# zhouxinlzu/PebbleSDR

Hardware: AMD Instinct MI355X
Metric: IQ Msamples/s through full ProcessBlock chain (higher is better)
Workload: dtype f32; 1 GPU; configs[1]: 20 Msps int8-shape IQ (values k/128, resident in HBM as float2), 1 channel/GPU, mixer+decimate(D=64)+WFM mono demod + 8192-bin SignalSpectrum per 2048-sample frame; frames_per_buffer=2048, spectrum_bins=8192, parallelism=independent channel per GPU, no collectives

## Files before the change

### pebblesdr_amd/csrc/fft_lds.h

```cpp
#pragma once
#include "common.h"

namespace pg {

__device__ __forceinline__ int lpad(int i) { return i + ((i >> 5) << 2); }
__device__ __forceinline__ int lpad4(int i) { return i + (i >> 4); }
__device__ __forceinline__ int lpad1(int i) { return i + (i >> 5); }
enum { kPad4per32 = 0, kPad1per16 = 1, kPad1per32 = 2 };
template <int A> __device__ __forceinline__ int lpad_sel(int i) { return A == kPad1per16 ? lpad4(i) : A == kPad1per32 ? lpad1(i) : lpad(i); }
template <int N> struct FftLds { static constexpr int kSlots = N + (N >> 5) * 4; };

__host__ __device__ constexpr int fft_passes(int n) { return n == 8192 ? 5 : 4; }
__host__ __device__ constexpr int fft_radix(int n, int pass) { return n == 2048 ? (pass == 0 ? 4 : 8) : n == 4096 ? 8 : (pass == 0 ? 2 : 8); }
__host__ __device__ constexpr int fft_tw_off(int n, int P)
{
    int off = 0, p = 1;
    for (int i = 0; i < fft_passes(n); i++) {
        if (p == P) return off;
        if (p > 1) off += 3 * p;
        p *= fft_radix(n, i);
    }
    return off;
}

template <int DIR> __device__ __forceinline__ float2 mul_mj(float2 a)
{
    return DIR > 0 ? make_float2(a.y, -a.x) : make_float2(-a.y, a.x);
}
template <int DIR> __device__ __forceinline__ float2 twid(float2 w)
{
    return DIR > 0 ? w : make_float2(w.x, -w.y);
}

template <int DIR> __device__ __forceinline__ void bfly2(float2 *u)
{
    float2 a = u[0], b = u[1];
    u[0] = cadd(a, b);
    u[1] = csub(a, b);
}
template <int DIR> __device__ __forceinline__ float2 add_mj(float2 a, float2 b)
{
    return cswap(b) * make_float2((float)DIR, (float)-DIR) + a;
}
template <int DIR> __device__ __forceinline__ float2 sub_mj(float2 a, float2 b)
{
    return cswap(b) * make_float2((float)-DIR, (float)DIR) + a;
}
template <int DIR> __device__ __forceinline__ void bfly4(float2 *u)
{
    float2 t0 = cadd(u[0], u[2]), t1 = csub(u[0], u[2]);
    float2 t2 = cadd(u[1], u[3]), d = csub(u[1], u[3]);
    u[0] = cadd(t0, t2);
    u[2] = csub(t0, t2);
    u[1] = add_mj<DIR>(t1, d);
    u[3] = sub_mj<DIR>(t1, d);
}
template <int DIR> __device__ __forceinline__ void bfly8(float2 *u)
{
    float2 e[4] = {u[0], u[2], u[4], u[6]};
    float2 o[4] = {u[1], u[3], u[5], u[7]};
    bfly4<DIR>(e);
    bfly4<DIR>(o);
    const float c = 0.70710678118654752440f;
    const float2 o1 = cscale(add_mj<DIR>(o[1], o[1]), c);
    const float2 o3 = cscale(sub_mj<DIR>(o[3], o[3]), c);
    u[0] = cadd(e[0], o[0]); u[4] = csub(e[0], o[0]);
    u[1] = cadd(e[1], o1);   u[5] = csub(e[1], o1);
    u[2] = add_mj<DIR>(e[2], o[2]); u[6] = sub_mj<DIR>(e[2], o[2]);
    u[3] = csub(e[3], o3);   u[7] = cadd(e[3], o3);
}
__host__ __device__ constexpr int perm32(int k) { return 4 * (k & 7) + (k >> 3); }
__device__ __forceinline__ void dft32(float2 *u)
{
    constexpr float kC[22] = {1.f, 0.98078528040323044913f, 0.92387953251128675613f, 0.83146961230254523708f, 0.70710678118654752440f,
                              0.55557023301960222474f, 0.38268343236508977173f, 0.19509032201612826785f, 0.f, -0.19509032201612826785f,
                              -0.38268343236508977173f, -0.55557023301960222474f, -0.70710678118654752440f, -0.83146961230254523708f,
                              -0.92387953251128675613f, -0.98078528040323044913f, -1.f, -0.98078528040323044913f, -0.92387953251128675613f,
                              -0.83146961230254523708f, -0.70710678118654752440f, -0.55557023301960222474f};
    constexpr float kS[22] = {0.f, -0.19509032201612826785f, -0.38268343236508977173f, -0.55557023301960222474f, -0.70710678118654752440f,
                              -0.83146961230254523708f, -0.92387953251128675613f, -0.98078528040323044913f, -1.f, -0.98078528040323044913f,
                              -0.92387953251128675613f, -0.83146961230254523708f, -0.70710678118654752440f, -0.55557023301960222474f,
                              -0.38268343236508977173f, -0.19509032201612826785f, 0.f, 0.19509032201612826785f, 0.38268343236508977173f,
                              0.55557023301960222474f, 0.70710678118654752440f, 0.83146961230254523708f};
#pragma unroll
    for (int nb = 0; nb < 4; nb++) {
        float2 t[8];
#pragma unroll
        for (int na = 0; na < 8; na++) t[na] = u[nb + 4 * na];
        bfly8<+1>(t);
#pragma unroll
        for (int ka = 0; ka < 8; ka++) {
            const int m = nb * ka;
            u[4 * ka + nb] = m == 0 ? t[ka] : m == 8 ? mul_mj<+1>(t[ka]) : cmul(make_float2(kC[m], kS[m]), t[ka]);
        }
    }
#pragma unroll
    for (int ka = 0; ka < 8; ka++) bfly4<+1>(u + 4 * ka);
}

template <int R, int DIR> __device__ __forceinline__ void bfly(float2 *u)
{
    if (R == 2) bfly2<DIR>(u);
    else if (R == 4) bfly4<DIR>(u);
    else bfly8<DIR>(u);
}

template <int T> __device__ __forceinline__ void fft_sync()
{
    if (T == 64) wave_sync();
    else __syncthreads();
}

template <int N, int T, int R, int P, int DIR, bool FIRST, bool LAST>
__device__ __forceinline__ void fft_pass(float2 (&x)[N / T], float2 *lds, const float2 *__restrict__ tw, int tid)
{
    constexpr int E = N / T, Q = E / R;
    static_assert(E % R == 0 && Q >= 1, "points per work-item must be a multiple of the radix");
    constexpr int PAD_IN = (!FIRST && P == 4) ? kPad1per16 : (!FIRST && T == 64 && P == 32) ? kPad1per32 : kPad4per32;
    constexpr int PAD_OUT = (FIRST && R == 4) ? kPad1per16 : kPad4per32;
    float2 w1 = make_float2(1.f, 0.f), w2 = w1, w4 = w1;
    auto fetch_tw = [&](int k) {
        if (T == 64) opaque(k);
        const float2 *t = tw + fft_tw_off(N, P) + k;
        w1 = twid<DIR>(t[0]);
        if (R >= 4) w2 = twid<DIR>(t[P]);
        if (R == 8) w4 = twid<DIR>(t[2 * P]);
    };
    if (P > 1) fetch_tw(tid & (P - 1));
    if (!FIRST) {
        {
            const float2 *rp = lds + lpad_sel<PAD_IN>(tid);
#pragma unroll
            for (int q = 0; q < Q; q += 2) {
#pragma unroll
                for (int r = 0; r < R; r++) {
                    x[q + r * Q] = rp[lpad_sel<PAD_IN>(T * (q + r * Q))];
                    if (q + 1 < Q) x[q + 1 + r * Q] = rp[lpad_sel<PAD_IN>(T * (q + 1 + r * Q))];
                }
                if (T == 64) sched_fence();
            }
        }
        fft_sync<T>();
    }
    const int jbase = (P <= T) ? (tid - (tid & (P - 1))) * R + (tid & (P - 1)) : tid;
    float2 *wbase = lds + lpad_sel<PAD_OUT>(jbase);
#pragma unroll
    for (int q = 0; q < Q; q++) {
        const int b = tid + T * q;
        float2 u[R];
#pragma unroll
        for (int r = 0; r < R; r++) u[r] = x[q + r * Q];
        const int k = b & (P - 1);
        if (P > 1) {
            if (P > T && q > 0) fetch_tw(k);
            u[1] = cmul(w1, u[1]);
            if (R >= 4) {
                const float2 w3 = cmul(w1, w2);
                u[2] = cmul(w2, u[2]);
                u[3] = cmul(w3, u[3]);
                if (R == 8) {
                    u[4] = cmul(w4, u[4]);
                    u[5] = cmul(cmul(w4, w1), u[5]);
                    u[6] = cmul(cmul(w4, w2), u[6]);
                    u[7] = cmul(cmul(w4, w3), u[7]);
                }
            }
        }
        bfly<R, DIR>(u);
        if (LAST) {
#pragma unroll
            for (int r = 0; r < R; r++) x[q + r * Q] = u[r];
        } else {
            const int cq = (P <= T) ? T * R * q : R * (T * q - (T * q) % P) + (T * q) % P;
            float2 *wp = wbase + lpad_sel<PAD_OUT>(cq);
#pragma unroll
            for (int r = 0; r < R; r++) wp[lpad_sel<PAD_OUT>(r * P)] = u[r];
        }
        if (T == 64) sched_fence();
    }
    if (!LAST) fft_sync<T>();
}

__device__ __forceinline__ void fft_first32(float2 (&x)[32], float2 *lds, int tid)
{
    dft32(x);
    float2 *wp = lds + lpad1(32 * tid);
#pragma unroll
    for (int k = 0; k < 32; k++) wp[k] = x[perm32(k)];
    wave_sync();
}

template <int N, int DIR, int T = 256>
__device__ __forceinline__ void fft_regs(float2 (&x)[N / T], float2 *lds, const float2 *__restrict__ tw, int tid)
{
    static_assert((T == 256 && (N == 2048 || N == 4096 || N == 8192)) || (T == 64 && N == 2048), "supported sizes");
    if (N == 2048 && T == 64) {
        static_assert(!(N == 2048 && T == 64) || DIR == +1, "the wave transform is forward only");
        fft_first32(reinterpret_cast<float2 (&)[32]>(x), lds, tid);
        fft_pass<N, T, 8, 32, DIR, false, false>(x, lds, tw, tid);
        fft_pass<N, T, 8, 256, DIR, false, true>(x, lds, tw, tid);
    } else if (N == 2048) {
        fft_pass<N, T, 4, 1, DIR, true, false>(x, lds, tw, tid);
        fft_pass<N, T, 8, 4, DIR, false, false>(x, lds, tw, tid);
        fft_pass<N, T, 8, 32, DIR, false, false>(x, lds, tw, tid);
        fft_pass<N, T, 8, 256, DIR, false, true>(x, lds, tw, tid);
    } else if (N == 4096) {
        fft_pass<N, T, 8, 1, DIR, true, false>(x, lds, tw, tid);
        fft_pass<N, T, 8, 8, DIR, false, false>(x, lds, tw, tid);
        fft_pass<N, T, 8, 64, DIR, false, false>(x, lds, tw, tid);
        fft_pass<N, T, 8, 512, DIR, false, true>(x, lds, tw, tid);
    } else {
        fft_pass<N, T, 2, 1, DIR, true, false>(x, lds, tw, tid);
        fft_pass<N, T, 8, 2, DIR, false, false>(x, lds, tw, tid);
        fft_pass<N, T, 8, 16, DIR, false, false>(x, lds, tw, tid);
        fft_pass<N, T, 8, 128, DIR, false, false>(x, lds, tw, tid);
        fft_pass<N, T, 8, 1024, DIR, false, true>(x, lds, tw, tid);
    }
}

}
```

### pebblesdr_amd/csrc/fft_t128.h

```cpp
#pragma once
#include "fft_lds.h"

namespace pg {

constexpr int kTw128B = 0, kTw128C = 48, kTw128Count = 48 + 512;

__host__ __device__ constexpr int perm16(int k) { return 4 * (k & 3) + (k >> 2); }

__device__ __forceinline__ void dft16(float2 *u)
{
    constexpr float kC[10] = {1.f, 0.92387953251128675613f, 0.70710678118654752440f, 0.38268343236508977173f, 0.f,
                              -0.38268343236508977173f, -0.70710678118654752440f, -0.92387953251128675613f, -1.f, -0.92387953251128675613f};
    constexpr float kS[10] = {0.f, -0.38268343236508977173f, -0.70710678118654752440f, -0.92387953251128675613f, -1.f,
                              -0.92387953251128675613f, -0.70710678118654752440f, -0.38268343236508977173f, 0.f, 0.38268343236508977173f};
#pragma unroll
    for (int nb = 0; nb < 4; nb++) {
        float2 t[4];
#pragma unroll
        for (int na = 0; na < 4; na++) t[na] = u[nb + 4 * na];
        bfly4<+1>(t);
#pragma unroll
        for (int ka = 0; ka < 4; ka++) {
            const int m = nb * ka;
            u[4 * ka + nb] = m == 0 ? t[ka] : m == 4 ? mul_mj<+1>(t[ka]) : cmul(make_float2(kC[m], kS[m]), t[ka]);
        }
    }
#pragma unroll
    for (int ka = 0; ka < 4; ka++) bfly4<+1>(u + 4 * ka);
}

struct Tw128Regs {
    float2 b1, b2, b4, c1, c2, c4, c8;
    float2 cx[16];
};
__device__ __forceinline__ void tw128_fill_cx(Tw128Regs &w)
{
    w.cx[0] = make_float2(1.f, 0.f);
    w.cx[1] = w.c1; w.cx[2] = w.c2; w.cx[3] = cmul_pk(w.c1, w.c2); w.cx[4] = w.c4;
    w.cx[5] = cmul_pk(w.c4, w.c1); w.cx[6] = cmul_pk(w.c4, w.c2); w.cx[7] = cmul_pk(w.c4, w.cx[3]); w.cx[8] = w.c8;
#pragma unroll
    for (int i = 1; i < 8; i++) w.cx[8 + i] = cmul_pk(w.c8, w.cx[i]);
}

template <class Sync, bool DO_LDS = true, bool DO_MATH = true, bool REGS = false, bool FULLC = false, int HELD = 0>
__device__ __forceinline__ void fft2048_t128(float2 (&x)[16], float2 *lds, const float2 *__restrict__ tw, int t, Sync sync, Tw128Regs wr = Tw128Regs())
{
    if (DO_MATH) dft16(x);
    if (DO_LDS) {
        float2 *wp = lds + lpad4(16 * t);
#pragma unroll
        for (int k = 0; k < 16; k++) wp[k] = x[perm16(k)];
    }
    sync();
    {
        const int k = t & 15;
        float2 w1, w2, w4;
        if (REGS) { w1 = wr.b1; w2 = wr.b2; w4 = wr.b4; }
        else { w1 = tw[kTw128B + k]; w2 = tw[kTw128B + 16 + k]; w4 = tw[kTw128B + 32 + k]; }
        if (DO_LDS) {
            const float2 *rp = lds + lpad4(t);
#pragma unroll
            for (int m = 0; m < 16; m++) x[m] = rp[136 * m];
        }
        sync();
        const float2 w3 = cmul_pk(w1, w2), w5 = cmul_pk(w4, w1), w6 = cmul_pk(w4, w2), w7 = cmul_pk(w4, w3);
        float2 *wbase = lds + lpad((t - k) * 8 + k);
#pragma unroll
        for (int q = 0; q < 2; q++) {
            float2 u[8];
#pragma unroll
            for (int r = 0; r < 8; r++) u[r] = x[q + 2 * r];
            if (DO_MATH) {
                u[1] = cmul_pk(w1, u[1]); u[2] = cmul_pk(w2, u[2]); u[3] = cmul_pk(w3, u[3]); u[4] = cmul_pk(w4, u[4]);
                u[5] = cmul_pk(w5, u[5]); u[6] = cmul_pk(w6, u[6]); u[7] = cmul_pk(w7, u[7]);
                bfly8<+1>(u);
            }
            float2 *wp = wbase + lpad(1024 * q);
            if (DO_LDS) {
#pragma unroll
                for (int r = 0; r < 8; r++) wp[lpad(16 * r)] = u[r];
            } else {
#pragma unroll
                for (int r = 0; r < 8; r++) x[q + 2 * r] = u[r];
            }
        }
    }
    sync();
    {
        float2 w1, w2, w4, w8;
        if (REGS) { w1 = wr.c1; w2 = wr.c2; w4 = wr.c4; w8 = wr.c8; }
        else { w1 = tw[kTw128C + t]; w2 = tw[kTw128C + 128 + t]; w4 = tw[kTw128C + 256 + t]; w8 = tw[kTw128C + 384 + t]; }
        if (DO_LDS) {
            const float2 *rp = lds + lpad(t);
#pragma unroll
            for (int m = 0; m < 16; m++) x[m] = rp[144 * m];
        }
        sync();
        if (!DO_MATH) return;
        if (REGS && FULLC) {
#pragma unroll
            for (int m = 1; m < 16; m++) x[m] = cmul_pk(wr.cx[m], x[m]);
        } else {
        const float2 w3 = cmul_pk(w1, w2), w5 = cmul_pk(w4, w1), w6 = cmul_pk(w4, w2), w7 = cmul_pk(w4, w3);
        x[1] = cmul_pk(w1, x[1]); x[2] = cmul_pk(w2, x[2]); x[3] = cmul_pk(w3, x[3]); x[4] = cmul_pk(w4, x[4]);
        x[5] = cmul_pk(w5, x[5]); x[6] = cmul_pk(w6, x[6]); x[7] = cmul_pk(w7, x[7]); x[8] = cmul_pk(w8, x[8]);
        x[9] = cmul_pk(REGS && HELD >= 1 ? wr.cx[9] : cmul_pk(w8, w1), x[9]);
        x[10] = cmul_pk(REGS && HELD >= 2 ? wr.cx[10] : cmul_pk(w8, w2), x[10]);
        x[11] = cmul_pk(REGS && HELD >= 3 ? wr.cx[11] : cmul_pk(w8, w3), x[11]);
        x[12] = cmul_pk(REGS && HELD >= 4 ? wr.cx[12] : cmul_pk(w8, w4), x[12]);
        x[13] = cmul_pk(REGS && HELD >= 5 ? wr.cx[13] : cmul_pk(w8, w5), x[13]);
        x[14] = cmul_pk(REGS && HELD >= 6 ? wr.cx[14] : cmul_pk(w8, w6), x[14]);
        x[15] = cmul_pk(REGS && HELD >= 7 ? wr.cx[15] : cmul_pk(w8, w7), x[15]);
        }
        dft16(x);
        float2 y[16];
#pragma unroll
        for (int r = 0; r < 16; r++) y[r] = x[perm16(r)];
#pragma unroll
        for (int r = 0; r < 16; r++) x[r] = y[r];
    }
}

}
```

### pebblesdr_amd/csrc/kernels_spectrum.h

```cpp
#pragma once
#include "fft_lds.h"
#include "fft_t128.h"
#include "fft_w64.h"
#include "hb_const.h"
#include "params.h"

namespace pg {

template <int ZP>
__global__ __launch_bounds__(256, 2) void k_spectrum(const float2 *__restrict__ in, float *__restrict__ out,
                                                      const float *__restrict__ window, const float2 *__restrict__ btab,
                                                      const float2 *__restrict__ tw_nf, const float *__restrict__ prev_in,
                                                      float *__restrict__ prev_out, SpectrumParams sp)
{
    constexpr int NF = 2048, E = NF / 64, BINS = NF * ZP, GROUPS = 4 / ZP, TG = 64 * ZP;
    constexpr int SL = NF / ZP, EL = E / ZP;
    constexpr int XOFF = NF / 2;
    constexpr int REGION = (XOFF + SL > FftLds<NF>::kSlots) ? XOFF + SL : FftLds<NF>::kSlots;
    __shared__ float2 lds[4][REGION];
    __shared__ float2 tw_lds[fft_tw_off(NF, NF)];
    const int tid = threadIdx.x, lane = tid & 63;
    const int wave = __builtin_amdgcn_readfirstlane(tid >> 6);
    const int g = wave / ZP, q = wave % ZP, s = blockIdx.y;
    const int G = sp.frames_per_group;
    const long long f0 = ((long long)blockIdx.x * GROUPS + g) * G;
    const float2 *x = in + (long long)s * sp.in_pitch;
    float *y = out + (long long)s * sp.out_pitch;
    float2 *my = lds[wave];
    float *stage = reinterpret_cast<float *>(my);

    for (int i = threadIdx.x; i < fft_tw_off(NF, NF); i += 256) tw_lds[i] = tw_nf[i];

    constexpr bool WIN_REGS = EL <= 8;
    float win[WIN_REGS ? EL : 1];
    if (WIN_REGS) {
#pragma unroll
        for (int i = 0; i < EL; i++) win[i] = window[q * SL + lane + 64 * i];
    }
    const float *wq = window + q * SL + lane;
    const float2 tw_lane = cis_cycles(-(double)(lane * q) / (double)BINS);
    const float2 *bq = btab + q * E;

    float pa[E];
    const float db_off = 6.02059991327962f * __builtin_amdgcn_logf(0.5f * sp.scale);
    float2 xn[EL];
    {
        const long long ff = f0 > 0 ? f0 - 1 : 0;
        if (ff < sp.n_frames) {
#pragma unroll
            for (int i = 0; i < EL; i++) xn[i] = x[ff * NF + q * SL + lane + 64 * i];
#pragma unroll
            for (int i = 0; i < EL; i++) my[XOFF + lane + 64 * i] = cscale(xn[i], WIN_REGS ? win[i] : wq[64 * i]);
        }
    }
    __syncthreads();

    for (int it = -1; it < G; it++) {
        const long long f = f0 + it;
        const bool live = f < sp.n_frames;
        const bool xform = live && f >= 0;
        int ln = lane;
        opaque(ln);
        const bool fetch = it + 1 < G && f + 1 < sp.n_frames && f >= 0;
        if (fetch) {
            const float2 *xp = x + (f + 1) * NF + q * SL + ln;
#pragma unroll
            for (int i = 0; i < EL; i++) xn[i] = xp[64 * i];
        }
        float2 v[E];
        if (xform) {
            const float2 *gp = &lds[g * ZP][XOFF + ln];
#pragma unroll
            for (int m = 0; m < E; m++) {
                const float2 xv = gp[((64 * m) / SL) * REGION + (64 * m) % SL];
                v[m] = ZP == 1 ? xv : cmul(bq[m], cmul(tw_lane, xv));
            }
        }
        __syncthreads();
        if (live && f < 0) {
            const float *pp = prev_in + (long long)s * BINS + ZP * ln + q;
#pragma unroll
            for (int m = 0; m < E; m++) pa[m] = pp[ZP * 64 * m];
        } else if (xform) {
            fft_regs<NF, +1, 64>(v, my, tw_lds, ln);
            float *st = stage + ln;
            float mag[E];
#pragma unroll
            for (int m = 0; m < E; m++) mag[m] = v[m].x * v[m].x + v[m].y * v[m].y;
#pragma unroll
            for (int m = 0; m < E; m++) mag[m] = __builtin_amdgcn_sqrtf(mag[m]);
            sched_fence();
#pragma unroll
            for (int m = 0; m < E; m++) {
                const float a = mag[m] + pa[m];
                pa[m] = mag[m];
                mag[m] = a;
            }
#pragma unroll
            for (int m = 0; m < E; m++) mag[m] = __builtin_amdgcn_logf(mag[m]);
            sched_fence();
#pragma unroll
            for (int m = 0; m < E; m++)
                st[64 * m] = fminf(fmaxf(fmaf(6.02059991327962f, mag[m], db_off), -120.f), 0.f);
            if (f == sp.n_frames - 1) {
                float *pp = prev_out + (long long)s * BINS + ZP * ln + q;
#pragma unroll
                for (int m = 0; m < E; m++) pp[ZP * 64 * m] = pa[m];
            }
        }
        __syncthreads();
        if (fetch) {
            float2 *xs = my + XOFF + ln;
#pragma unroll
            for (int i = 0; i < EL; i++) xs[64 * i] = cscale(xn[i], WIN_REGS ? win[i] : wq[64 * i]);
        }
        if (it >= 0 && live) {
            const int tg = ln + 64 * q;
            const float *sp0 = reinterpret_cast<const float *>(lds[g * ZP]) + tg;
            float *yf = y + f * (long long)BINS;
#pragma unroll
            for (int i = 0; i < NF / TG; i++) {
                const int j = tg + TG * i;
                float db[ZP];
#pragma unroll
                for (int qq = 0; qq < ZP; qq++) db[qq] = sp0[qq * (REGION * 2) + TG * i];
                const int u = (ZP * j + BINS / 2) & (BINS - 1);
                if (ZP == 4) store_stream(reinterpret_cast<float4 *>(yf + u), make_float4(db[0], db[1], db[2], db[3]));
                else if (ZP == 2) store_stream(reinterpret_cast<float2 *>(yf + u), make_float2(db[0], db[1]));
                else store_stream(yf + u, db[0]);
            }
        }
        __syncthreads();
    }
}

struct DecLds {
    float2 z0[14 + 256], z1[22 + 128], z2[2][46 + 64], xt[2][10];
};

template <int HALVES, int FMT, bool DEC = false, bool FULLC = false>
static __global__ __launch_bounds__(512 * HALVES, 2 * HALVES) void k_spectrum_t128(const float2 *__restrict__ in, float *__restrict__ out,
                                                                 const float *__restrict__ window, const float2 *__restrict__ btab128,
                                                                 const float2 *__restrict__ tw128, const float *__restrict__ prev_in,
                                                                 float *__restrict__ prev_out, SpectrumParams sp, int shift, RawSrc raw,
                                                                 DecFuse df)
{
    constexpr int NF = 2048, ZP = 4, BINS = NF * ZP, E = 16, SL = NF / ZP;
    constexpr int REGION = FftLds<NF>::kSlots;
    constexpr int HELD = (DEC || FULLC) ? 0 : (FMT == 3 ? 5 : FMT >= 0 ? 7 : 6);
    constexpr int XOFF = NF / 2 + (DEC ? 16 : 0), RSTEP = DEC ? 144 : 128;
    auto fslot = [](int m) { return XOFF + m + (DEC ? (m >> 3) : 0); };
    constexpr bool RAW = FMT >= 0;
    __shared__ float2 lds_all[HALVES][4][REGION];
    __shared__ DecLds dec_all[DEC ? HALVES : 1];
    __builtin_amdgcn_s_setprio(3);
    const int tid = threadIdx.x & 511, lane = tid & 63;
    const int half = HALVES > 1 ? __builtin_amdgcn_readfirstlane(threadIdx.x >> 9) : 0;
    float2 (*lds)[REGION] = lds_all[half];
    DecLds &dl = dec_all[DEC ? half : 0];
    const int wave = __builtin_amdgcn_readfirstlane(tid >> 6);
    const int q = wave >> 1, s = blockIdx.y;
    const int G = sp.frames_per_group;
    const long long f0 = ((long long)blockIdx.x * HALVES + half) * G;
    const float2 *x = in + (long long)s * sp.in_pitch;
    float *y = out + (long long)s * sp.out_pitch;
    float2 *my = lds[q];
    float *stage = reinterpret_cast<float *>(my);
    float win[4];
#pragma unroll
    for (int i = 0; i < 4; i++) win[i] = RAW ? window[4 * tid + i] : window[tid + 512 * i];
    const int t0 = (wave & 1) * 64 + lane;
    const float2 *bq = btab128 + q * E;
    Tw128Regs twr;
    {
        const float2 *tq = tw128 + q * kTw128Count;
        const int kb = t0 & 15;
        twr.b1 = tq[kTw128B + kb]; twr.b2 = tq[kTw128B + 16 + kb]; twr.b4 = tq[kTw128B + 32 + kb];
        twr.c1 = tq[kTw128C + t0]; twr.c2 = tq[kTw128C + 128 + t0]; twr.c4 = tq[kTw128C + 256 + t0]; twr.c8 = tq[kTw128C + 384 + t0];
        if (FULLC || HELD > 0) tw128_fill_cx(twr);
    }
    const float db_off = 6.02059991327962f * __builtin_amdgcn_logf(0.5f * sp.scale);
    float pa[E];
    float2 xn[4];
    RawQuad<FMT < 0 ? 0 : FMT> xr;
    constexpr int kD[7] = {0, 2, 4, 5, 6, 8, 10};
    if (DEC) {
        for (int i = tid; i < (int)(sizeof(DecLds) / sizeof(float2)); i += 512) reinterpret_cast<float2 *>(&dl)[i] = make_float2(0.f, 0.f);
    }
    float2 c0n[7], phn;
    auto dec_prefetch = [&](int td2) {
#pragma unroll
        for (int i = 0; i < 7; i++) c0n[i] = make_float2(0.f, 0.f);
        phn = make_float2(0.f, 0.f);
        if (td2 < 256) {
#pragma unroll
            for (int i = 0; i < 7; i++) c0n[i] = df.c0tab[256 * i + td2];
            phn = df.ph_scratch[((long long)blockIdx.x * HALVES + half) * 256 + td2];
        }
    };
    if (DEC) dec_prefetch(tid);
    auto park = [&](int tt) {
        if (RAW) raw_convert4<FMT < 0 ? 0 : FMT>(raw, xr, xn);
#pragma unroll
        for (int i = 0; i < 4; i++) {
            const int reg = RAW ? tt >> 7 : i, m = RAW ? (4 * tt + i) & 511 : tt;
            const float2 v = cscale(xn[i], win[i]);
            lds[reg][fslot(m)] = v;
            if (DEC && m >= 502 && reg < 3) lds[reg + 1][fslot(m - 512)] = v;
        }
    };
    {
        const long long ff = f0 > 0 ? f0 - 1 : 0;
        if (DEC && f0 == 0) {
#pragma unroll
            for (int i = 0; i < 4; i++) {
                const float2 v = df.xtail[tid + 512 * i];
                lds[i][fslot(tid)] = v;
                if (tid >= 502 && i < 3) lds[i + 1][fslot(tid - 512)] = v;
            }
        } else if (ff < sp.n_frames) {
            if (RAW) {
                raw_fetch4<FMT < 0 ? 0 : FMT>(raw, (long long)s * sp.in_pitch + ff * NF + 4 * tid, xr);
            } else {
#pragma unroll
                for (int i = 0; i < 4; i++) xn[i] = x[ff * NF + tid + 512 * i];
            }
            park(tid);
        }
    }
    __syncthreads();
    if (HALVES > 1 && half == 1)
        for (int i = 0; i < shift; i++) __syncthreads();
    auto iteration = [&](const int it, float (&pa)[E], float (&pn)[E]) __attribute__((always_inline)) {
        const long long f = f0 + it;
        const bool live = f < sp.n_frames;
        const bool xform = live && f >= 0;
        int t = t0, td = tid;
        opaque(t);
        opaque(td);
        const bool fetch = it + 1 < G && f + 1 < sp.n_frames && (f >= 0 || DEC);
        auto fetch_next = [&]() {
            if (!fetch) return;
            if (RAW) {
                raw_fetch4<FMT < 0 ? 0 : FMT>(raw, (long long)s * sp.in_pitch + (f + 1) * NF + 4 * td, xr);
            } else {
                const float2 *xp = x + (f + 1) * NF + td;
#pragma unroll
                for (int i = 0; i < 4; i++) xn[i] = xp[512 * i];
            }
        };
        if (!DEC) fetch_next();
        float2 v[E];
        if (xform) {
            const float2 *gp = &lds[0][fslot(t)];
#pragma unroll
            for (int m = 0; m < E; m++) {
                const float2 xv = gp[(m / 4) * REGION + (m % 4) * RSTEP];
                v[m] = m == 0 ? xv : cmul(bq[m], xv);
            }
        }
        const bool dec_run = DEC && live;
        const bool dec_emit = dec_run && it >= 0;
        const int par = (int)(f & 1);
        if (dec_run) {
            if (td < 256) {
                float2 ph = make_float2(df.gain0, 0.f);
                if (df.mix_on) {
                    ph = ((it + 1) & 7) == 0 ? cscale(cis_cycles(df.phase0 + (double)((long long)NF * f + 8 * td - 9) * df.inc), df.a_inf * df.gain0) : cmul(df.wfr, phn);
                    df.ph_scratch[((long long)blockIdx.x * HALVES + half) * 256 + td] = ph;
                }
                const float2 *fb = &lds[td >> 6][XOFF + 9 * (td & 63)];
                v2f_t acc = {0.f, 0.f};
#pragma unroll
                for (int i = 0; i < 7; i++) {
                    const int c = kD[i] - 10, n = 8 * td + c;
                    const float2 xs = n >= 0 ? fb[c + (c >> 3)] : dl.xt[par ^ 1][n + 10];
                    acc = cmac_pk(acc, v2f_t{c0n[i].x, c0n[i].y}, v2f_t{xs.x, xs.y});
                }
                const float2 y0 = cmul(ph, make_float2(acc.x, acc.y));
                dl.z0[14 + td] = y0;
                if (dec_emit && f == sp.n_frames - 1) df.y0_tail[td] = y0;
            } else if (td < 266) {
                dl.xt[par][td - 256] = lds[3][fslot(502 + td - 256)];
            }
        }
        auto hb47 = [&](long long fr, bool emit) {
            const int m = (td - 448) & 31, part = (td - 448) >> 5;
            const float2 *z = dl.z2[(int)(fr & 1)];
            const float2 *w = z + 2 * m + 46 * part;
            const int sg = 1 - 2 * part;
            float2 acc = cscale(z[2 * m + 23], part ? 0.f : hb_tap<47>(23));
#pragma unroll
            for (int p = 0; p < 24; p += 2) acc = cadd(acc, cscale(w[sg * p], hb_tap<47>(p)));
            acc.x += __shfl_down(acc.x, 32);
            acc.y += __shfl_down(acc.y, 32);
            if (emit && part == 0) df.y[32 * fr + m] = cscale(acc, df.gain_last);
        };
        auto dec_slot = [&](int k) {
            if (k == 1) {
                if (dec_run && td >= 256 && td < 384) {
                    const int m = td - 256;
                    const float2 *w = dl.z0 + 2 * m;
                    float2 acc = cscale(w[7], hb_tap<15>(7));
#pragma unroll
                    for (int p = 0; p < 15; p += 2) acc = cadd(acc, cscale(w[p], hb_tap<15>(p)));
                    dl.z1[22 + m] = acc;
                }
                if (DEC && td >= 448 && it >= 1 && f - 1 < sp.n_frames) hb47(f - 1, true);
            } else if (k == 2) {
                if (!dec_run) return;
                if (td >= 384 && td < 448) {
                    const int m = td - 384;
                    const float2 *w = dl.z1 + 2 * m;
                    float2 acc = cscale(w[11], hb_tap<23>(11));
#pragma unroll
                    for (int p = 0; p < 23; p += 2) acc = cadd(acc, cscale(w[p], hb_tap<23>(p)));
                    dl.z2[par][46 + m] = acc;
                    if (m >= 18) dl.z2[par ^ 1][m - 18] = acc;
                } else if (td >= 448 && td < 462) {
                    dl.z0[td - 448] = dl.z0[256 + td - 448];
                }
            } else if (k == 3) {
                if (dec_run && td >= 384 && td < 406) dl.z1[td - 384] = dl.z1[128 + td - 384];
            }
        };
        if (DEC) fetch_next();
        __syncthreads();
        if (live && f < 0) {
            const float *pp = prev_in + (long long)s * BINS + ZP * t + q;
#pragma unroll
            for (int m = 0; m < E; m++) pa[m] = pp[ZP * 128 * m];
        }
        if (xform) {
            int slot = 0;
            auto bar = [&] {
                __syncthreads();
                if (DEC) dec_slot(++slot);
            };
            fft2048_t128<decltype(bar), true, true, true, FULLC, HELD>(v, my, tw128, t, bar, twr);
            float *st = stage + t;
            float mag[E];
#pragma unroll
            for (int m = 0; m < E; m++) mag[m] = v[m].x * v[m].x + v[m].y * v[m].y;
#pragma unroll
            for (int m = 0; m < E; m++) mag[m] = __builtin_amdgcn_sqrtf(mag[m]);
#pragma unroll
            for (int m = 0; m < E; m++) {
                const float a = mag[m] + pa[m];
                pn[m] = mag[m];
                mag[m] = a;
            }
#pragma unroll
            for (int m = 0; m < E; m++) mag[m] = __builtin_amdgcn_logf(mag[m]);
#pragma unroll
            for (int m = 0; m < E; m++) st[128 * m] = fminf(fmaxf(fmaf(6.02059991327962f, mag[m], db_off), -120.f), 0.f);
            if (f == sp.n_frames - 1) {
                float *pp = prev_out + (long long)s * BINS + ZP * t + q;
#pragma unroll
                for (int m = 0; m < E; m++) pp[ZP * 128 * m] = pn[m];
            }
        } else {
            if (HALVES > 1 || DEC) {
#pragma unroll
                for (int i = 0; i < 4; i++) {
                    __syncthreads();
                    if (DEC) dec_slot(i + 1);
                }
            }
            if (!DEC) {
#pragma unroll
                for (int m = 0; m < E; m++) pn[m] = pa[m];
            }
        }
        __syncthreads();
        if (DEC) dec_prefetch(td);
        if (fetch) park(td);
        if (DEC && fetch && f + 1 == sp.n_frames - 1) {
#pragma unroll
            for (int i = 0; i < 4; i++) {
                const int n = RAW ? 4 * td + i : td + 512 * i;
                df.xtail_next[n] = cscale(xn[i], win[i]);
            }
        }
        if (it >= 0 && live) {
            float *yf = y + f * (long long)BINS;
            int j[NF / 512];
#pragma unroll
            for (int i = 0; i < NF / 512; i++) {
                j[i] = td + 512 * i;
                opaque(j[i]);
            }
            float4 d[NF / 512];
#pragma unroll
            for (int i = 0; i < NF / 512; i++) {
                const float *spi = reinterpret_cast<const float *>(lds[0]) + j[i];
                d[i].x = spi[0 * (REGION * 2)];
                d[i].y = spi[1 * (REGION * 2)];
                d[i].z = spi[2 * (REGION * 2)];
                d[i].w = spi[3 * (REGION * 2)];
            }
#pragma unroll
            for (int i = 0; i < NF / 512; i++) {
                const int u = (ZP * j[i] + BINS / 2) & (BINS - 1);
                store_stream(reinterpret_cast<float4 *>(yf + u), d[i]);
            }
        }
        __syncthreads();
    };
    if (DEC) {
        for (int it = -1; it < G; it++) iteration(it, pa, pa);
    } else {
        float pb[E];
        for (int it = -1; it < G; it += 2) {
            iteration(it, pa, pb);
            if (it + 1 >= G) break;
            iteration(it + 1, pb, pa);
        }
    }
    if (DEC) {
        const long long fl = f0 + G - 1;
        if (tid >= 448 && fl < sp.n_frames) {
            const int m = (tid - 448) & 31, part = (tid - 448) >> 5;
            const float2 *z = dl.z2[(int)(fl & 1)];
            const float2 *w = z + 2 * m + 46 * part;
            const int sg = 1 - 2 * part;
            float2 acc = cscale(z[2 * m + 23], part ? 0.f : hb_tap<47>(23));
#pragma unroll
            for (int p = 0; p < 24; p += 2) acc = cadd(acc, cscale(w[sg * p], hb_tap<47>(p)));
            acc.x += __shfl_down(acc.x, 32);
            acc.y += __shfl_down(acc.y, 32);
            if (part == 0) df.y[32 * fl + m] = cscale(acc, df.gain_last);
        }
    }
    if (HALVES > 1 && half == 0)
        for (int i = 0; i < shift; i++) __syncthreads();
}

template <int FMT>
static __global__ __launch_bounds__(256, 2) void k_spectrum_w64(const float2 *__restrict__ in, float *__restrict__ out, const float *__restrict__ window,
                                                                 const float2 *__restrict__ btab, const float *__restrict__ prev_in,
                                                                 float *__restrict__ prev_out, SpectrumParams sp, RawSrc raw)
{
    constexpr int NF = 2048, ZP = 4, BINS = NF * ZP, E = 32, QSTRIDE = kW64ImageSlots * 2;
    constexpr bool RAW = FMT >= 0;
    __shared__ float2 frame[NF];
    __shared__ float2 img[ZP][kW64ImageSlots];
    __shared__ float2 stab[ZP][32];
    const int tid = threadIdx.x, lane = tid & 63;
    const int q = __builtin_amdgcn_readfirstlane(tid >> 6), s = blockIdx.y;
    const int G = sp.frames_per_group;
    const long long f0 = (long long)blockIdx.x * G;
    const float2 *x = in + (long long)s * sp.in_pitch;
    float *y = out + (long long)s * sp.out_pitch;
    const W64Consts c = w64_consts(lane, cis_cycles(-(double)(lane * q) / (double)BINS));
    const float db_off = 6.02059991327962f * __builtin_amdgcn_logf(0.5f * sp.scale);
    const int kb = w64_kbase(lane);
    if (tid < ZP * 32) stab[tid >> 5][tid & 31] = btab[tid];
    float pa[E];
    float2 xn[8];
    float win[8];
#ifdef PG_W64_PROFILE
    long long tacc[8] = {0, 0, 0, 0, 0, 0, 0, 0}, tl = 0;
#define PG_W64_TICK(i) { const long long t_ = __builtin_readcyclecounter(); tacc[i] += t_ - tl; tl = t_; }
#else
#define PG_W64_TICK(i)
#endif
    auto fetch_window = [&](int td) {
#pragma unroll
        for (int i = 0; i < 8; i++) win[i] = RAW ? window[4 * td + 1024 * (i >> 2) + (i & 3)] : window[td + 256 * i];
    };
    auto fetch_frame = [&](long long ff, int td) {
        if (RAW) {
            const long long i0 = (long long)s * sp.in_pitch + ff * NF + 4 * td;
            float2 a[4], b[4];
            raw_load4<FMT < 0 ? 0 : FMT>(raw, i0, a);
            raw_load4<FMT < 0 ? 0 : FMT>(raw, i0 + 1024, b);
#pragma unroll
            for (int i = 0; i < 4; i++) { xn[i] = a[i]; xn[4 + i] = b[i]; }
        } else {
            const float2 *xp = x + ff * NF + td;
#pragma unroll
            for (int i = 0; i < 8; i++) xn[i] = xp[256 * i];
        }
    };
    auto park = [&](int td) {
#pragma unroll
        for (int i = 0; i < 8; i++) frame[RAW ? 4 * td + 1024 * (i >> 2) + (i & 3) : td + 256 * i] = cscale(xn[i], win[i]);
    };
    {
        const long long ff = f0 > 0 ? f0 - 1 : 0;
        if (ff < sp.n_frames) {
            fetch_frame(ff, tid);
            fetch_window(tid);
            park(tid);
        }
    }
    __syncthreads();
#ifdef PG_W64_PROFILE
    tl = __builtin_readcyclecounter();
#endif
    for (int it = -1; it < G; it++) {
        const long long f = f0 + it;
        const bool live = f < sp.n_frames;
        const bool xform = live && f >= 0;
        int ln = lane, td = tid, qq = q;
        opaque(ln);
        opaque(td);
        asm volatile("" : "+s"(qq));
        const bool fetch = it + 1 < G && f + 1 < sp.n_frames && f >= 0;
        const long long fnext = f + 1 < sp.n_frames ? (f + 1 > 0 ? f + 1 : 0) : sp.n_frames - 1;
        fetch_frame(fnext, td);
        if (live && f < 0) {
            int kq = ZP * kb + q;
            opaque(kq);
            const float *pp = prev_in + (long long)s * BINS + kq;
#pragma unroll
            for (int h = 0; h < 2; h++)
#pragma unroll
                for (int k3 = 0; k3 < 16; k3++) pa[16 * h + perm16(k3)] = pp[ZP * (32 * h + 128 * k3)];
        }
        if (xform) {
            float2 v[E];
            const float2 *gp = frame + ln;
            const float2 *sq = stab[qq];
            v[0] = gp[0];
#pragma unroll
            for (int m = 1; m < E; m++) v[m] = cmul_pk(sq[m], gp[64 * m]);
            PG_W64_TICK(0)
            fft2048_w64(v, img[q], c, ln);
            PG_W64_TICK(1)
            sched_fence();
            fetch_window(td);
            sched_fence();
            float *st = reinterpret_cast<float *>(img[q]) + w64_kbase(ln);
#pragma unroll
            for (int g = 0; g < 4; g++) {
                constexpr int NG = 8;
                const int h = g >> 1, kk = (g & 1) * NG;
                float mag[NG];
#pragma unroll
                for (int m = 0; m < NG; m++) {
                    const float2 z = v[16 * h + perm16(kk + m)];
                    mag[m] = z.x * z.x + z.y * z.y;
                }
#pragma unroll
                for (int m = 0; m < NG; m++) mag[m] = __builtin_amdgcn_sqrtf(mag[m]);
#pragma unroll
                for (int m = 0; m < NG; m++) {
                    const float a = mag[m] + pa[16 * h + perm16(kk + m)];
                    pa[16 * h + perm16(kk + m)] = mag[m];
                    mag[m] = a;
                }
#pragma unroll
                for (int m = 0; m < NG; m++) mag[m] = __builtin_amdgcn_logf(mag[m]);
#pragma unroll
                for (int m = 0; m < NG; m++)
                    st[32 * h + 128 * (kk + m)] = fminf(fmaxf(fmaf(6.02059991327962f, mag[m], db_off), -120.f), 0.f);
                sched_fence();
            }
            if (f == sp.n_frames - 1) {
                int kq = ZP * kb + q;
                opaque(kq);
// ... 707 lines not shown
```

Measured before the change: 127,200 Msamples/s.

## Transpose first FFT LDS stage and issue LDS gathers as batched inline-asm reads

Changes the first write/read exchange of the 2048-point t128 FFT to a transposed layout with pitch 130, so each thread writes strided and reads 16 consecutive-stride-8 slots. It adds a helper that issues sixteen ds_read_b64 with immediate offsets in inline asm followed by a single lgkmcnt wait, and uses it for the FFT stage reads and the frame gather in the spectrum kernel. The goal is to cut address arithmetic and bank conflicts and to keep all LDS loads in flight together. The volatile asm with a full wait limits compiler scheduling and may add register pressure, and the new layout is the default (PAIR_READS=false).

After: 128,600 Msamples/s (median of 6 runs). +1.1%, better.

```diff
diff --git a/pebblesdr_amd/csrc/fft_lds.h b/pebblesdr_amd/csrc/fft_lds.h
--- a/pebblesdr_amd/csrc/fft_lds.h
+++ b/pebblesdr_amd/csrc/fft_lds.h
@@ -3,12 +3,50 @@
 
 namespace pg {
 
-__device__ __forceinline__ int lpad(int i) { return i + ((i >> 5) << 2); }
-__device__ __forceinline__ int lpad4(int i) { return i + (i >> 4); }
-__device__ __forceinline__ int lpad1(int i) { return i + (i >> 5); }
+__host__ __device__ constexpr int lpad(int i) { return i + ((i >> 5) << 2); }
+__host__ __device__ constexpr int lpad4(int i) { return i + (i >> 4); }
+__host__ __device__ constexpr int lpad1(int i) { return i + (i >> 5); }
 enum { kPad4per32 = 0, kPad1per16 = 1, kPad1per32 = 2 };
-template <int A> __device__ __forceinline__ int lpad_sel(int i) { return A == kPad1per16 ? lpad4(i) : A == kPad1per32 ? lpad1(i) : lpad(i); }
+template <int A> __host__ __device__ constexpr int lpad_sel(int i) { return A == kPad1per16 ? lpad4(i) : A == kPad1per32 ? lpad1(i) : lpad(i); }
 template <int N> struct FftLds { static constexpr int kSlots = N + (N >> 5) * 4; };
+
+template <int S> struct LdsStride { static constexpr int at(int m) { return S * m; } };
+__device__ __forceinline__ unsigned lds_addr(const void *p)
+{
+    return (unsigned)(uintptr_t)(__attribute__((address_space(3))) const void *)p;
+}
+template <class OFF, int I0> __device__ __forceinline__ void lds_read8_b64(v2f_t *r, unsigned a)
+{
+    asm volatile("ds_read_b64 %0, %8 offset:%9\n\tds_read_b64 %1, %8 offset:%10\n\tds_read_b64 %2, %8 offset:%11\n\tds_read_b64 %3, %8 offset:%12\n\t"
+                 "ds_read_b64 %4, %8 offset:%13\n\tds_read_b64 %5, %8 offset:%14\n\tds_read_b64 %6, %8 offset:%15\n\tds_read_b64 %7, %8 offset:%16"
+                 : "=&v"(r[I0]), "=&v"(r[I0 + 1]), "=&v"(r[I0 + 2]), "=&v"(r[I0 + 3]), "=&v"(r[I0 + 4]), "=&v"(r[I0 + 5]), "=&v"(r[I0 + 6]), "=&v"(r[I0 + 7])
+                 : "v"(a), "n"(8 * OFF::at(I0)), "n"(8 * OFF::at(I0 + 1)), "n"(8 * OFF::at(I0 + 2)), "n"(8 * OFF::at(I0 + 3)), "n"(8 * OFF::at(I0 + 4)),
+                   "n"(8 * OFF::at(I0 + 5)), "n"(8 * OFF::at(I0 + 6)), "n"(8 * OFF::at(I0 + 7))
+                 : "memory");
+}
+template <int I0, bool WAIT> __device__ __forceinline__ void lds_tie8(v2f_t *r)
+{
+    if (WAIT)
+        asm volatile("s_waitcnt lgkmcnt(0)" : "+v"(r[I0]), "+v"(r[I0 + 1]), "+v"(r[I0 + 2]), "+v"(r[I0 + 3]), "+v"(r[I0 + 4]), "+v"(r[I0 + 5]), "+v"(r[I0 + 6]), "+v"(r[I0 + 7])::"memory");
+    else
+        asm volatile("" : "+v"(r[I0]), "+v"(r[I0 + 1]), "+v"(r[I0 + 2]), "+v"(r[I0 + 3]), "+v"(r[I0 + 4]), "+v"(r[I0 + 5]), "+v"(r[I0 + 6]), "+v"(r[I0 + 7]));
+}
+template <int N, class OFF> __device__ __forceinline__ void lds_gather_b64(float2 (&x)[N], const float2 *p)
+{
+    static_assert(N % 8 == 0 && N <= 32 && 8 * OFF::at(N - 1) + 8 <= 65536, "blocks of eight reads, 16-bit byte offsets");
+    const unsigned a = lds_addr(p);
+    v2f_t r[N];
+    lds_read8_b64<OFF, 0>(r, a);
+    if (N > 8) lds_read8_b64<OFF, (N > 8 ? 8 : 0)>(r, a);
+    if (N > 16) lds_read8_b64<OFF, (N > 16 ? 16 : 0)>(r, a);
+    if (N > 24) lds_read8_b64<OFF, (N > 24 ? 24 : 0)>(r, a);
+    lds_tie8<0, true>(r);
+    if (N > 8) lds_tie8<(N > 8 ? 8 : 0), false>(r);
+    if (N > 16) lds_tie8<(N > 16 ? 16 : 0), false>(r);
+    if (N > 24) lds_tie8<(N > 24 ? 24 : 0), false>(r);
+#pragma unroll
+    for (int m = 0; m < N; m++) x[m] = make_float2(r[m].x, r[m].y);
+}
 
 __host__ __device__ constexpr int fft_passes(int n) { return n == 8192 ? 5 : 4; }
 __host__ __device__ constexpr int fft_radix(int n, int pass) { return n == 2048 ? (pass == 0 ? 4 : 8) : n == 4096 ? 8 : (pass == 0 ? 2 : 8); }
diff --git a/pebblesdr_amd/csrc/fft_t128.h b/pebblesdr_amd/csrc/fft_t128.h
--- a/pebblesdr_amd/csrc/fft_t128.h
+++ b/pebblesdr_amd/csrc/fft_t128.h
@@ -6,6 +6,9 @@
 constexpr int kTw128B = 0, kTw128C = 48, kTw128Count = 48 + 512;
 
 __host__ __device__ constexpr int perm16(int k) { return 4 * (k & 3) + (k >> 2); }
+constexpr int kT128Pitch = 130;
+__host__ __device__ constexpr int t128_slot_ab(int e) { return kT128Pitch * (e & 15) + (e >> 4); }
+static_assert(t128_slot_ab(2047) < FftLds<2048>::kSlots, "the transposed image fits the padded one");
 
 __device__ __forceinline__ void dft16(float2 *u)
 {
@@ -42,14 +45,20 @@
     for (int i = 1; i < 8; i++) w.cx[8 + i] = cmul_pk(w.c8, w.cx[i]);
 }
 
-template <class Sync, bool DO_LDS = true, bool DO_MATH = true, bool REGS = false, bool FULLC = false, int HELD = 0>
+template <class Sync, bool DO_LDS = true, bool DO_MATH = true, bool REGS = false, bool FULLC = false, int HELD = 0, bool PAIR_READS = false>
 __device__ __forceinline__ void fft2048_t128(float2 (&x)[16], float2 *lds, const float2 *__restrict__ tw, int t, Sync sync, Tw128Regs wr = Tw128Regs())
 {
     if (DO_MATH) dft16(x);
     if (DO_LDS) {
-        float2 *wp = lds + lpad4(16 * t);
+        if (PAIR_READS) {
+            float2 *wp = lds + lpad4(16 * t);
 #pragma unroll
-        for (int k = 0; k < 16; k++) wp[k] = x[perm16(k)];
+            for (int k = 0; k < 16; k++) wp[k] = x[perm16(k)];
+        } else {
+            float2 *wp = lds + t;
+#pragma unroll
+            for (int k = 0; k < 16; k++) wp[kT128Pitch * k] = x[perm16(k)];
+        }
     }
     sync();
     {
@@ -58,9 +67,13 @@
         if (REGS) { w1 = wr.b1; w2 = wr.b2; w4 = wr.b4; }
         else { w1 = tw[kTw128B + k]; w2 = tw[kTw128B + 16 + k]; w4 = tw[kTw128B + 32 + k]; }
         if (DO_LDS) {
-            const float2 *rp = lds + lpad4(t);
+            if (PAIR_READS) {
+                const float2 *rp = lds + lpad4(t);
 #pragma unroll
-            for (int m = 0; m < 16; m++) x[m] = rp[136 * m];
+                for (int m = 0; m < 16; m++) x[m] = rp[136 * m];
+            } else {
+                lds_gather_b64<16, LdsStride<8>>(x, lds + t128_slot_ab(t));
+            }
         }
         sync();
         const float2 w3 = cmul_pk(w1, w2), w5 = cmul_pk(w4, w1), w6 = cmul_pk(w4, w2), w7 = cmul_pk(w4, w3);
@@ -92,8 +105,12 @@
         else { w1 = tw[kTw128C + t]; w2 = tw[kTw128C + 128 + t]; w4 = tw[kTw128C + 256 + t]; w8 = tw[kTw128C + 384 + t]; }
         if (DO_LDS) {
             const float2 *rp = lds + lpad(t);
+            if (PAIR_READS) {
 #pragma unroll
-            for (int m = 0; m < 16; m++) x[m] = rp[144 * m];
+                for (int m = 0; m < 16; m++) x[m] = rp[144 * m];
+            } else {
+                lds_gather_b64<16, LdsStride<144>>(x, rp);
+            }
         }
         sync();
         if (!DO_MATH) return;
diff --git a/pebblesdr_amd/csrc/kernels_spectrum.h b/pebblesdr_amd/csrc/kernels_spectrum.h
--- a/pebblesdr_amd/csrc/kernels_spectrum.h
+++ b/pebblesdr_amd/csrc/kernels_spectrum.h
@@ -136,6 +136,9 @@
 
 struct DecLds {
     float2 z0[14 + 256], z1[22 + 128], z2[2][46 + 64], xt[2][10];
+};
+template <int REGION, int RSTEP> struct FrameGatherOff {
+    static constexpr int at(int m) { return (m / 4) * REGION + (m % 4) * RSTEP; }
 };
 
 template <int HALVES, int FMT, bool DEC = false, bool FULLC = false>
@@ -252,12 +255,9 @@
         if (!DEC) fetch_next();
         float2 v[E];
         if (xform) {
-            const float2 *gp = &lds[0][fslot(t)];
-#pragma unroll
-            for (int m = 0; m < E; m++) {
-                const float2 xv = gp[(m / 4) * REGION + (m % 4) * RSTEP];
-                v[m] = m == 0 ? xv : cmul(bq[m], xv);
-            }
+            lds_gather_b64<E, FrameGatherOff<REGION, RSTEP>>(v, &lds[0][fslot(t)]);
+#pragma unroll
+            for (int m = 1; m < E; m++) v[m] = cmul(bq[m], v[m]);
         }
         const bool dec_run = DEC && live;
         const bool dec_emit = dec_run && it >= 0;
```
